# basilevh/tcow

Hardware: AMD Instinct MI355X
Metric: train clips/sec (T=30, 240x320) (higher is better)
Workload: dtype bf16; 1 GPU; TCOW Seeker train step: T=30 240x320 patch16, 12-layer divided space-time ViT (D=768), num_queries=3, causal_attention=1, 1 clip/GPU; clips_per_gpu=1, num_queries=3, parallelism=dp1, optimizer=AdamW lr 1e-4, clip 0.3

## Files before the change

### tcow_amd/csrc/gemm_bf16.hip

```cpp
#include <stdlib.h>

#include "common.h"
#include "gemm_nt_common.h"

namespace {

constexpr int BM = 128, BN = 128;
constexpr int BK = 64;
constexpr int TILE_BYTES = BM * 128;
constexpr int STAGE_BYTES = 2 * TILE_BYTES;
constexpr int NT_LDS_BYTES = 2 * STAGE_BYTES;

__device__ __forceinline__ void nt_epilogue(const NtParams& p, char* smem, f32x16 (&acc)[2][2], float4 b4, int tid, int wm, int wn, int l31, int hi, int m0, int n0) {
    const int c4 = (tid & 31) * 4, gn = n0 + c4;
    const bool col_ok = gn < p.N;
    float* ct = reinterpret_cast<float*>(smem);
#pragma unroll
    for (int i = 0; i < 2; ++i)
#pragma unroll
        for (int j = 0; j < 2; ++j)
#pragma unroll
            for (int r = 0; r < 16; ++r) {
                const int row = wm * 64 + i * 32 + crow32(r, hi);
                const int col = wn * 64 + j * 32 + l31;
// ... 584 lines not shown
    const int mbeg = z * p.mps;
    const int mend = (mbeg + p.mps < p.M) ? mbeg + p.mps : p.M;

    const int lrow = lane >> 5, cl = lane & 31;
    const bf16_t* zero = reinterpret_cast<const bf16_t*>(&g_zero16);
    int ycol[2], xcol[2];
#pragma unroll
    for (int e = 0; e < 2; ++e) {
        const int r3 = (e << 1) | lrow;
        const int sc = cl ^ (r3 << 2);
        ycol[e] = n0 + sc * 8; xcol[e] = k0 + sc * 8;
    }
    f32x16 acc[4][2];
#pragma unroll
    for (int i = 0; i < 4; ++i)
#pragma unroll
        for (int j = 0; j < 2; ++j)
#pragma unroll
            for (int r = 0; r < 16; ++r) acc[i][j][r] = 0.f;

    auto issue = [&](int mt, int stage) {
        char* sy = smem + stage * T2_STAGE;
        char* sx = sy + T2_TILE;
#pragma unroll
        for (int j = 0; j < 4; ++j) {
            const int q = wave * 4 + j;
            const int gm = mt + q * 2 + lrow;
            const bool ok = gm < mend;
            const bf16_t* ys = (ok && ycol[j & 1] < p.N) ? p.dY + (size_t)gm * p.ldy + ycol[j & 1] : zero;
            const bf16_t* xs = (ok && xcol[j & 1] < p.K) ? p.X + (size_t)gm * p.ldx + xcol[j & 1] : zero;
            glds16(ys, sy + q * 1024);
            glds16(xs, sx + q * 1024);
        }
    };
    const bool interior = n0 + T2 <= p.N && k0 + T2 <= p.K;
    typedef int i32x4_ __attribute__((ext_vector_type(4)));
    auto make_srd = [](const void* base, long bytes) {
        const uint64_t b = (uint64_t)(uintptr_t)base;
        i32x4_ r; r[0] = (int)(uint32_t)b; r[1] = (int)(uint32_t)((b >> 32) & 0xffffu); r[2] = (int)(uint32_t)bytes; r[3] = 0x00020000;
        return r;
    };
    const i32x4_ srd_y = make_srd(p.dY, ((long)(p.M - 1) * p.ldy + p.N) * 2), srd_x = make_srd(p.X, ((long)(p.M - 1) * p.ldx + p.K) * 2);
    const uint32_t yv0 = (uint32_t)(lrow * p.ldy + ycol[0]) * 2u, yv1 = (uint32_t)(lrow * p.ldy + ycol[1]) * 2u;
    const uint32_t xv0 = (uint32_t)(lrow * p.ldx + xcol[0]) * 2u, xv1 = (uint32_t)(lrow * p.ldx + xcol[1]) * 2u;
    const bool small32 = (long)p.M * p.ldy < (1L << 29) && (long)p.M * p.ldx < (1L << 29);
    const uint32_t lds_base = (uint32_t)(uintptr_t)(LDS_PTR(char))smem;
#define TN_BLD(voff, srd, soff, ldsdst) \
    asm volatile("s_mov_b32 m0, %3\n\ts_nop 0\n\tbuffer_load_dwordx4 %0, %1, %2 offen lds" :: "v"(voff), "s"(srd), "s"(soff), "s"(ldsdst) : "memory")
    auto issue_fast = [&](int mt, int stage) {
        const uint32_t dy = lds_base + stage * T2_STAGE + wave * 4096, dx = dy + T2_TILE;
        const uint32_t sy = (uint32_t)((long)(mt + wave * 8) * p.ldy * 2), sx = (uint32_t)((long)(mt + wave * 8) * p.ldx * 2);
        const uint32_t ry = (uint32_t)(2 * p.ldy * 2), rx = (uint32_t)(2 * p.ldx * 2);
        TN_BLD(yv0, srd_y, sy, dy); TN_BLD(xv0, srd_x, sx, dx);
        TN_BLD(yv1, srd_y, sy + ry, dy + 1024); TN_BLD(xv1, srd_x, sx + rx, dx + 1024);
        TN_BLD(yv0, srd_y, sy + 2 * ry, dy + 2048); TN_BLD(xv0, srd_x, sx + 2 * rx, dx + 2048);
        TN_BLD(yv1, srd_y, sy + 3 * ry, dy + 3072); TN_BLD(xv1, srd_x, sx + 3 * rx, dx + 3072);
    };
    const int q16 = lane & 15, g16 = (lane >> 4) & 1, hi = lane >> 5;
    const int rr = 8 * hi + (q16 >> 2);
    int y_off[4], x_off[2];
#pragma unroll
    for (int i = 0; i < 4; ++i) {
        const int cy = wm * 128 + i * 32 + 16 * g16 + 4 * (q16 & 3);
        y_off[i] = rr * T2_ROWB + ((((cy >> 3) ^ ((q16 >> 2) << 2))) << 4) + (cy & 7) * 2;
    }
#pragma unroll
    for (int j = 0; j < 2; ++j) {
        const int cx = wn * 64 + j * 32 + 16 * g16 + 4 * (q16 & 3);
        x_off[j] = rr * T2_ROWB + ((((cx >> 3) ^ ((q16 >> 2) << 2))) << 4) + (cx & 7) * 2;
    }

    const int cs_col = tid & 255;
    const int cs_lo = pk * p.rows_per_pk, cs_hi = (cs_lo + p.rows_per_pk < T2_MC) ? cs_lo + p.rows_per_pk : T2_MC;
    const int cs_chunk = tid & 31, cs_rg = tid >> 5;
    float csum[8] = {0.f, 0.f, 0.f, 0.f, 0.f, 0.f, 0.f, 0.f};

    const int nmt = (mend - mbeg + T2_MC - 1) / T2_MC;
    auto issue_stage = [&](int st_, int buf_) {
        const int mt = mbeg + st_ * T2_MC;
        if (interior && small32 && (mt + T2_MC <= mend || mend == p.M)) issue_fast(mt, buf_); else issue(mt, buf_);
    };
    if constexpr (SCHED >= 2) {
        if (nmt > 0) {
            issue_fast(mbeg, 0);
            if (nmt > 1) { issue_fast(mbeg + T2_MC, 1); asm volatile("s_waitcnt vmcnt(8)" ::: "memory"); }
            else asm volatile("s_waitcnt vmcnt(0)" ::: "memory");
            __syncthreads();
        }
    } else if (nmt > 0) {
        issue(mbeg, 0);
        if (SCHED == 1 && nmt > 1) { issue_stage(1, 1); asm volatile("s_waitcnt vmcnt(8)" ::: "memory"); }
        else asm volatile("s_waitcnt vmcnt(0)" ::: "memory");
        __syncthreads();
    }
    typedef uint32_t u32x2 __attribute__((ext_vector_type(2)));
    typedef uint32_t u32x4 __attribute__((ext_vector_type(4)));
    const uint32_t lds0 = (uint32_t)(uintptr_t)(LDS_PTR(char))smem;
    uint32_t ya[4], xa[2];
#pragma unroll
    for (int i = 0; i < 4; ++i) ya[i] = lds0 + (uint32_t)y_off[i];
#pragma unroll
    for (int j = 0; j < 2; ++j) xa[j] = lds0 + (uint32_t)x_off[j];
    u32x2 fyl[2][4], fyh[2][4], fxl[2][2], fxh[2][2];
    u32x4 kfrag = (u32x4){1u, 2u, 3u, 4u};
    if (AB & 128) asm volatile("" : "+v"(kfrag));
    u32x4 kfy[2][4], kfx[2][2];
    if (AB & 512) {
#pragma unroll
        for (int b = 0; b < 2; ++b) {
#pragma unroll
            for (int i = 0; i < 4; ++i) {
                kfy[b][i] = (u32x4){1u, 2u, 3u, 4u};
                if (AB & 1024) {
#pragma unroll
                    for (int c = 0; c < 4; ++c) { uint32_t h = (uint32_t)(tid * 97 + b * 31 + i * 7 + c) * 2654435761u; kfy[b][i][c] = (h & 0x807f807fu) | 0x3f003f00u | ((h >> 3) & 0x00800080u); }
                }
                asm volatile("" : "+v"(kfy[b][i]));
            }
#pragma unroll
            for (int j = 0; j < 2; ++j) {
                kfx[b][j] = (u32x4){1u, 2u, 3u, 4u};
                if (AB & 1024) {
#pragma unroll
                    for (int c = 0; c < 4; ++c) { uint32_t h = (uint32_t)(tid * 89 + b * 29 + j * 5 + c + 1000) * 2654435761u; kfx[b][j][c] = (h & 0x807f807fu) | 0x3f003f00u | ((h >> 3) & 0x00800080u); }
                }
                asm volatile("" : "+v"(kfx[b][j]));
            }
        }
    }
#define TCOW_TRR(dst, addr, off) asm volatile("ds_read_b64_tr_b16 %0, %1 offset:%2" : "=v"(dst) : "v"(addr), "i"(off))
#define TCOW_TN_READ(buf, ks, so)                                                                                          \
    do {                                                                                                                   \
        if (AB & 16) break;                                                                                                \
        _Pragma("unroll") for (int j = 0; j < 2; ++j) {                                                                    \
            TCOW_TRR(fxl[buf][j], xa[j] + (so), T2_TILE + (ks) * 16 * T2_ROWB);                                            \
            TCOW_TRR(fxh[buf][j], xa[j] + (so), T2_TILE + (ks) * 16 * T2_ROWB + 4 * T2_ROWB);                              \
        }                                                                                                                  \
        _Pragma("unroll") for (int i = 0; i < 4; ++i) {                                                                    \
            TCOW_TRR(fyl[buf][i], ya[i] + (so), (ks) * 16 * T2_ROWB);                                                      \
            TCOW_TRR(fyh[buf][i], ya[i] + (so), (ks) * 16 * T2_ROWB + 4 * T2_ROWB);                                        \
        }                                                                                                                  \
    } while (0)
#define TCOW_TN_FRAG(lo, hi) ((AB & 128) ? __builtin_bit_cast(bf16x8, kfrag) : __builtin_bit_cast(bf16x8, (u32x4){(lo).x, (lo).y, (hi).x, (hi).y}))
#define TCOW_TN_MFMA8(buf)                                                                                                 \
    if (!(AB & 32)) _Pragma("unroll") for (int i = 0; i < 4; ++i)                                                          \
        _Pragma("unroll") for (int j = 0; j < 2; ++j)                                                                      \
            acc[i][j] = TCOW_MFMA_32x32x16_H16(TCOW_TN_FRAG(fyl[buf][i], fyh[buf][i]), TCOW_TN_FRAG(fxl[buf][j], fxh[buf][j]), acc[i][j], 0, 0, 0)

    if (nmt > 0) TCOW_TN_READ(0, 0, 0u);
    if (AB & 16) {
#pragma unroll
        for (int b = 0; b < 2; ++b) {
#pragma unroll
            for (int j = 0; j < 2; ++j) { fxl[b][j] = (u32x2){1u, 2u}; fxh[b][j] = (u32x2){3u, 4u}; }
#pragma unroll
            for (int i = 0; i < 4; ++i) { fyl[b][i] = (u32x2){5u, 6u}; fyh[b][i] = (u32x2){7u, 8u}; }
        }
    }
    if constexpr (SCHED == 2) {
#define TN_BLDA(...) do { if (!(AB & 2)) TN_BLD(__VA_ARGS__); } while (0)
#define TN_RDA(...) do { if (!(AB & 16)) TCOW_TRR(__VA_ARGS__); } while (0)
#define TN_NOP do { } while (0)
#define TN_MF(cur, i, j) if (!(AB & 32)) acc[i][j] = TCOW_MFMA_32x32x16_H16((AB & 512) ? __builtin_bit_cast(bf16x8, kfy[cur][i]) : TCOW_TN_FRAG(fyl[cur][i], fyh[cur][i]), (AB & 512) ? __builtin_bit_cast(bf16x8, kfx[cur][j]) : TCOW_TN_FRAG(fxl[cur][j], fxh[cur][j]), acc[i][j], 0, 0, 0); \
                    __builtin_amdgcn_sched_barrier(0)
#define TN_BLK(cur, nxt, OFFK, son, W0, B0, B1, B2, B3, B4, B5, B6, B7)                                                                  \
    do {                                                                                                                                 \
        if (!(AB & 256)) asm volatile("s_waitcnt lgkmcnt(" #W0 ")" ::: "memory"); __builtin_amdgcn_sched_barrier(0);                     \
        TN_MF(cur, 0, 0); TN_RDA(fxl[nxt][0], xa[0] + (son), T2_TILE + (OFFK)); TN_RDA(fxh[nxt][0], xa[0] + (son), T2_TILE + (OFFK) + 4 * T2_ROWB); B0; \
        TN_MF(cur, 0, 1); TN_RDA(fxl[nxt][1], xa[1] + (son), T2_TILE + (OFFK)); TN_RDA(fxh[nxt][1], xa[1] + (son), T2_TILE + (OFFK) + 4 * T2_ROWB); B1; \
        TN_MF(cur, 1, 0); TN_RDA(fyl[nxt][0], ya[0] + (son), (OFFK)); TN_RDA(fyh[nxt][0], ya[0] + (son), (OFFK) + 4 * T2_ROWB); B2;              \
        TN_MF(cur, 1, 1); TN_RDA(fyl[nxt][1], ya[1] + (son), (OFFK)); TN_RDA(fyh[nxt][1], ya[1] + (son), (OFFK) + 4 * T2_ROWB); B3;              \
        if (!(AB & 256)) asm volatile("s_waitcnt lgkmcnt(10)" ::: "memory"); __builtin_amdgcn_sched_barrier(0);     \
        TN_MF(cur, 2, 0); TN_RDA(fyl[nxt][2], ya[2] + (son), (OFFK)); TN_RDA(fyh[nxt][2], ya[2] + (son), (OFFK) + 4 * T2_ROWB); B4;              \
        TN_MF(cur, 2, 1); TN_RDA(fyl[nxt][3], ya[3] + (son), (OFFK)); TN_RDA(fyh[nxt][3], ya[3] + (son), (OFFK) + 4 * T2_ROWB); B5;              \
        if (!(AB & 256)) asm volatile("s_waitcnt lgkmcnt(12)" ::: "memory"); __builtin_amdgcn_sched_barrier(0);      \
        TN_MF(cur, 3, 0); B6;                                                                                                            \
        TN_MF(cur, 3, 1); B7;                                                                                                            \
    } while (0)
        for (int it = 0; it < nmt; ++it) {
            const int stage = it & 1;
            const uint32_t so = (uint32_t)stage * T2_STAGE;
            const char* sy = smem + stage * T2_STAGE;
            TN_BLK(0, 1, 1 * 16 * T2_ROWB, so, 4, TN_NOP, TN_NOP, TN_NOP, TN_NOP, TN_NOP, TN_NOP, TN_NOP, TN_NOP);
            TN_BLK(1, 0, 2 * 16 * T2_ROWB, so, 4, TN_NOP, TN_NOP, TN_NOP, TN_NOP, TN_NOP, TN_NOP, TN_NOP, TN_NOP);
            TN_BLK(0, 1, 3 * 16 * T2_ROWB, so, 4, TN_NOP, TN_NOP, TN_NOP, TN_NOP, TN_NOP, TN_NOP, TN_NOP, TN_NOP);
            if (p.bias_part && !(AB & 64)) {
#pragma unroll
                for (int u = 0; u < 4; ++u) {
                    const int r = cs_lo + cs_rg + 16 * u;
                    if (r < cs_hi) {
                        const uint4 v = *reinterpret_cast<const uint4*>(sy + r * T2_ROWB + ((cs_chunk ^ ((r & 3) << 2)) << 4));
                        csum[0] += bflo(v.x); csum[1] += bfhi(v.x); csum[2] += bflo(v.y); csum[3] += bfhi(v.y);
                        csum[4] += bflo(v.z); csum[5] += bfhi(v.z); csum[6] += bflo(v.w); csum[7] += bfhi(v.w);
                    }
                }
            }
            asm volatile("s_waitcnt vmcnt(0) lgkmcnt(0)" ::: "memory");
            if (!(AB & 4)) __syncthreads();
            {
                const int mt2 = mbeg + (it + 2) * T2_MC;
                const bool more = it + 2 < nmt;
                const uint32_t dy = lds_base + so + wave * 4096, dx = dy + T2_TILE;
                const uint32_t by = (uint32_t)((long)(mt2 + wave * 8) * p.ldy * 2), bx = (uint32_t)((long)(mt2 + wave * 8) * p.ldx * 2);
                const uint32_t yw0 = more ? yv0 : 0x80000000u, yw1 = more ? yv1 : 0x80000000u;
                const uint32_t xw0 = more ? xv0 : 0x80000000u, xw1 = more ? xv1 : 0x80000000u;
                const uint32_t ry = (uint32_t)(2 * p.ldy * 2), rx = (uint32_t)(2 * p.ldx * 2);
                const uint32_t sn = so ^ (uint32_t)T2_STAGE;
                TN_BLK(1, 0, 0, sn, 0, TN_BLDA(yw0, srd_y, by, dy), TN_BLDA(xw0, srd_x, bx, dx), TN_BLDA(yw1, srd_y, by + ry, dy + 1024),
                       TN_BLDA(xw1, srd_x, bx + rx, dx + 1024), TN_BLDA(yw0, srd_y, by + 2 * ry, dy + 2048), TN_BLDA(xw0, srd_x, bx + 2 * rx, dx + 2048),
                       TN_BLDA(yw1, srd_y, by + 3 * ry, dy + 3072), TN_BLDA(xw1, srd_x, bx + 3 * rx, dx + 3072));
            }
        }
#undef TN_BLK
#undef TN_MF
#undef TN_NOP
#undef TN_BLDA
#undef TN_RDA
    } else
    if constexpr (SCHED == 1) {
        for (int it = 0; it < nmt; ++it) {
            const int stage = it & 1;
            const uint32_t so = (uint32_t)stage * T2_STAGE;
            const char* sy = smem + stage * T2_STAGE;
            TCOW_TN_READ(1, 1, so);
            asm volatile("s_waitcnt lgkmcnt(12)" ::: "memory");
            __builtin_amdgcn_sched_barrier(0);
            TCOW_TN_MFMA8(0);
            TCOW_TN_READ(0, 2, so);
            asm volatile("s_waitcnt lgkmcnt(12)" ::: "memory");
            __builtin_amdgcn_sched_barrier(0);
            TCOW_TN_MFMA8(1);
            TCOW_TN_READ(1, 3, so);
            asm volatile("s_waitcnt lgkmcnt(12)" ::: "memory");
            __builtin_amdgcn_sched_barrier(0);
            TCOW_TN_MFMA8(0);
            if (p.bias_part && !(AB & 64)) {
#pragma unroll
                for (int u = 0; u < 4; ++u) {
                    const int r = cs_lo + cs_rg + 16 * u;
                    if (r < cs_hi) {
                        const uint4 v = *reinterpret_cast<const uint4*>(sy + r * T2_ROWB + ((cs_chunk ^ ((r & 3) << 2)) << 4));
                        csum[0] += bflo(v.x); csum[1] += bfhi(v.x); csum[2] += bflo(v.y); csum[3] += bfhi(v.y);
                        csum[4] += bflo(v.z); csum[5] += bfhi(v.z); csum[6] += bflo(v.w); csum[7] += bfhi(v.w);
                    }
                }
            }
            asm volatile("s_waitcnt vmcnt(0) lgkmcnt(0)" ::: "memory");
            if (!(AB & 4)) __syncthreads();
            if (it + 2 < nmt && !(AB & 2)) issue_stage(it + 2, stage);
            if (it + 1 < nmt) TCOW_TN_READ(0, 0, so ^ (uint32_t)T2_STAGE);
            __builtin_amdgcn_sched_barrier(0);
            TCOW_TN_MFMA8(1);
        }
    }
    asm volatile("s_waitcnt lgkmcnt(0)"
                 : "+v"(fxl[0][0]), "+v"(fxl[0][1]), "+v"(fxh[0][0]), "+v"(fxh[0][1]), "+v"(fyl[0][0]), "+v"(fyl[0][1]), "+v"(fyl[0][2]), "+v"(fyl[0][3]),
                   "+v"(fyh[0][0]), "+v"(fyh[0][1]), "+v"(fyh[0][2]), "+v"(fyh[0][3])
                 :: "memory");
    __builtin_amdgcn_sched_barrier(0);
#undef TCOW_TRR
#undef TCOW_TN_READ
#undef TCOW_TN_FRAG
#undef TCOW_TN_MFMA8
    if (p.bias_part) {
        float* red = reinterpret_cast<float*>(smem);
        __syncthreads();
#pragma unroll
        for (int e = 0; e < 8; ++e) red[cs_rg * 256 + cs_chunk * 8 + e] = csum[e];
        __syncthreads();
        if (n0 + cs_col < p.N) {
            float t = 0.f;
            if (tid < 256) {
#pragma unroll
                for (int g = 0; g < 16; ++g) t += red[g * 256 + cs_col];
            }
            p.bias_part[(((size_t)z * p.tiles_k + pk) * 2 + (tid >> 8)) * p.N + n0 + cs_col] = t;
        }
        __syncthreads();
    }

    if (AB & 8) {
#pragma unroll
        for (int i = 0; i < 4; ++i)
#pragma unroll
            for (int j = 0; j < 2; ++j) asm volatile("" :: "v"(acc[i][j]));
        return;
    }
    float* out = p.slab + (size_t)z * p.N * p.K;
    const int l31 = lane & 31;
#pragma unroll
    for (int i = 0; i < 4; ++i)
#pragma unroll
        for (int j = 0; j < 2; ++j) {
            const int gk = k0 + wn * 64 + j * 32 + l31;
            if (gk >= p.K) continue;
#pragma unroll
            for (int r = 0; r < 16; ++r) {
                const int gn = n0 + wm * 128 + i * 32 + crow32(r, hi);
                if (gn < p.N) out[(size_t)gn * p.K + gk] = acc[i][j][r];
            }
        }
}

template <int SCHED>
__global__ __launch_bounds__(512, 2) void gemm_tn_bf16_256_kernel(TnParams p) {
    extern __shared__ __attribute__((aligned(16))) char smem[];
    tn256_body<0, SCHED>(p, xcd_remap(blockIdx.x, gridDim.x), smem);
}

constexpr int TN_GROUP_MAX = 40;
struct TnGroup { int n; int first[TN_GROUP_MAX + 1]; TnParams p[TN_GROUP_MAX]; };
template <int SCHED>
__global__ __launch_bounds__(512, 2) void gemm_tn_bf16_256_group_kernel(TnGroup g) {
    extern __shared__ __attribute__((aligned(16))) char smem[];
    const int pid = xcd_remap(blockIdx.x, gridDim.x);
    int k = 0;
    while (k + 1 < g.n && pid >= g.first[k + 1]) ++k;
    const TnParams p = g.p[k];
    tn256_body<0, SCHED>(p, pid - g.first[k], smem);
}

}

int tcow_tn_splits_256(int M, int N, int K) {
    const int tiles = cdiv(N, T2) * cdiv(K, T2);
    int s = 256 / tiles;
    const int max_s = M / 256;
    if (s > max_s) s = max_s;
    if (s > 64) s = 64;
    if (s < 1) s = 1;
    return s;
}
bool tcow_tn_use_256(int M, int N, int K) {
    const int tiles = cdiv(N, T2) * cdiv(K, T2);
    return M >= 4096 && N >= 256 && K >= 256 && tiles >= 9 && tiles <= 256;
}

static int tn_sched() { return 2; }
static bool tn_whole(int M, int N, int K, long ldy, long ldx) { return N % T2 == 0 && K % T2 == 0 && (long)M * ldy < (1L << 29) && (long)M * ldx < (1L << 29); }

int tcow_gemm_tn_bf16(hipStream_t stream, int M, int N, int K, const bf16_t* dY, long ldy, const bf16_t* X, long ldx, float* slab, int splits,
                      int* nz_out, float* bias_part, int* bias_parts_out) {
    TCOW_CHECK_ARG(N % 8 == 0 && K % 8 == 0 && ldy % 8 == 0 && ldx % 8 == 0, "tcow_gemm_tn(bf16): N, K, ldy, ldx must be multiples of 8");
    TnParams p;
    p.M = M; p.N = N; p.K = K; p.dY = dY; p.ldy = ldy; p.X = X; p.ldx = ldx; p.slab = slab;
    p.tiles_n = cdiv(N, TN_T); p.tiles_k = cdiv(K, TN_T);
    constexpr int mc = 32;
    int mps = cdiv(M, splits); mps = ((mps + 63) / 64) * 64;
    p.mps = mps;
    const int nz = cdiv(M, mps);
    p.nz = nz;
    *nz_out = nz;
    p.bias_part = bias_part;
    p.rows_per_pk = cdiv(mc, p.tiles_k);
    if (bias_parts_out) *bias_parts_out = nz * p.tiles_k * 2;
    if (tcow_tn_use_256(M, N, K)) {
        p.tiles_n = cdiv(N, T2); p.tiles_k = cdiv(K, T2);
        p.rows_per_pk = cdiv(T2_MC, p.tiles_k);
        if (bias_parts_out) *bias_parts_out = nz * p.tiles_k * 2;
        const int sched = (tn_sched() >= 2 && !tn_whole(M, N, K, ldy, ldx)) ? 1 : tn_sched();
#define TN_LAUNCH(S)                                                                                                       \
    do {                                                                                                                   \
        tcow_ensure_lds(reinterpret_cast<const void*>(gemm_tn_bf16_256_kernel<S>), T2_LDS);                                \
        hipLaunchKernelGGL(gemm_tn_bf16_256_kernel<S>, dim3(nz * p.tiles_n * p.tiles_k), dim3(512), T2_LDS, stream, p);    \
    } while (0)
        if (sched == 2) TN_LAUNCH(2); else TN_LAUNCH(1);
#undef TN_LAUNCH
        TCOW_CHECK_LAUNCH();
        return TCOW_OK;
    }
    const dim3 grid(8 * cdiv(nz, 8) * p.tiles_n * p.tiles_k);
    hipLaunchKernelGGL(gemm_tn_bf16_kernel<32>, grid, dim3(256), 32768, stream, p);
    TCOW_CHECK_LAUNCH();
    return TCOW_OK;
}

int tcow_tn_group_max(void) { return TN_GROUP_MAX; }
bool tcow_tn_group_ok(int n, const tcow_tn_problem* pr) {
    if (n < 2 || n > TN_GROUP_MAX) return false;
    for (int i = 0; i < n; ++i) {
        if (pr[i].M != pr[0].M || !tcow_tn_use_256(pr[i].M, pr[i].N, pr[i].K)) return false;
        if (pr[i].N % 8 || pr[i].K % 8 || pr[i].ldy % 8 || pr[i].ldx % 8) return false;
    }
    return true;
}
int tcow_tn_group_slices(int n, const tcow_tn_problem* pr) {
    int tiles = 0;
    for (int i = 0; i < n; ++i) tiles += cdiv(pr[i].N, T2) * cdiv(pr[i].K, T2);
    int max_s = pr[0].M / 256; if (max_s > 64) max_s = 64; if (max_s < 1) max_s = 1;
    int best = 1; double best_cost = 1e30;
    for (int s = 1; s <= max_s; ++s) {
        const int wg = s * tiles, rounds = cdiv(wg, 256);
        const double cost = (rounds * 256.0) / (double)wg + 0.044 * s;
        if (cost < best_cost - 1e-9) { best_cost = cost; best = s; }
    }
    return best;
}
int tcow_gemm_tn_bf16_group(hipStream_t stream, int n, const tcow_tn_problem* pr, int nz_req, float* const* slabs, float* const* bias_parts, int* nz_out,
                            int* bias_nparts) {
    TnGroup g;
    g.n = n;
    int first = 0, nz = 0;
    for (int i = 0; i < n; ++i) {
        TnParams& p = g.p[i];
        p.M = pr[i].M; p.N = pr[i].N; p.K = pr[i].K; p.dY = (const bf16_t*)pr[i].dY; p.ldy = pr[i].ldy; p.X = (const bf16_t*)pr[i].X; p.ldx = pr[i].ldx;
        p.slab = slabs[i];
        p.tiles_n = cdiv(p.N, T2); p.tiles_k = cdiv(p.K, T2);
        int mps = cdiv(p.M, nz_req); mps = ((mps + 63) / 64) * 64;
        p.mps = mps; p.nz = cdiv(p.M, mps); nz = p.nz;
        p.bias_part = bias_parts[i];
        p.rows_per_pk = cdiv(T2_MC, p.tiles_k);
        bias_nparts[i] = p.nz * p.tiles_k * 2;
        g.first[i] = first;
        first += p.nz * p.tiles_n * p.tiles_k;
    }
    g.first[n] = first;
    for (int i = n + 1; i <= TN_GROUP_MAX; ++i) g.first[i] = first;
    *nz_out = nz;
    int sched = tn_sched();
    for (int i = 0; i < n && sched >= 2; ++i) if (!tn_whole(pr[i].M, pr[i].N, pr[i].K, pr[i].ldy, pr[i].ldx)) sched = 1;
#define TN_LAUNCH(S)                                                                                                       \
    do {                                                                                                                   \
        tcow_ensure_lds(reinterpret_cast<const void*>(gemm_tn_bf16_256_group_kernel<S>), T2_LDS);                          \
        hipLaunchKernelGGL(gemm_tn_bf16_256_group_kernel<S>, dim3(first), dim3(512), T2_LDS, stream, g);                   \
    } while (0)
    if (sched == 2) TN_LAUNCH(2); else TN_LAUNCH(1);
#undef TN_LAUNCH
    TCOW_CHECK_LAUNCH();
    return TCOW_OK;
}
```

Measured before the change: 36.72 clips/s.

## Add phased ping-pong schedule for 256-tile TN weight-gradient GEMM

Adds a new tn256_phased body for the weight-gradient (TN) GEMM. It splits each K-stage into four phases that interleave transposed LDS reads (ds_read_b64_tr_b16), buffer loads for the next stage and 16x16x32 MFMA bursts. The two wave groups are staggered by an extra barrier, and the MFMA bursts run at raised priority. The default schedule switches from 2 to 3, so all whole-tile TN launches use it. This is meant to overlap memory and matrix work better than the old body, at the cost of heavier barrier choreography and a fragile vmcnt-based ordering.

Result: no change. 36.81 clips/s (median of 6 runs) (+0.2%).

```diff
diff --git a/tcow_amd/csrc/gemm_bf16.hip b/tcow_amd/csrc/gemm_bf16.hip
--- a/tcow_amd/csrc/gemm_bf16.hip
+++ b/tcow_amd/csrc/gemm_bf16.hip
@@ -910,10 +910,222 @@
         }
 }
 
+template <int AB>
+__device__ __forceinline__ void tn256_phased(const TnParams& p, const int pid, char* smem) {
+    const int tid = threadIdx.x, lane = tid & 63;
+    const int wave = __builtin_amdgcn_readfirstlane(tid >> 6);
+    const int wm = wave >> 2, wn = wave & 3;
+    const int ntile = p.tiles_n * p.tiles_k;
+    const int z = pid / ntile, tile = pid - z * ntile;
+    const int pn = tile / p.tiles_k, pk = tile - pn * p.tiles_k;
+    const int n0 = pn * T2, k0 = pk * T2;
+    const int mbeg = z * p.mps;
+    const int mend = (mbeg + p.mps < p.M) ? mbeg + p.mps : p.M;
+    const int nmt = (mend - mbeg + T2_MC - 1) / T2_MC;
+
+    typedef int i32x4_ __attribute__((ext_vector_type(4)));
+    typedef uint32_t u32x2 __attribute__((ext_vector_type(2)));
+    typedef uint32_t u32x4 __attribute__((ext_vector_type(4)));
+    auto make_srd = [](const void* base, long bytes) {
+        const uint64_t b = (uint64_t)(uintptr_t)base;
+        i32x4_ r; r[0] = (int)(uint32_t)b; r[1] = (int)(uint32_t)((b >> 32) & 0xffffu); r[2] = (int)(uint32_t)bytes; r[3] = 0x00020000;
+        return r;
+    };
+    const i32x4_ srd_y = make_srd(p.dY, ((long)(p.M - 1) * p.ldy + p.N) * 2), srd_x = make_srd(p.X, ((long)(p.M - 1) * p.ldx + p.K) * 2);
+    const int lrow = lane >> 5, cl = lane & 31;
+    uint32_t yv[2], xv[2];
+#pragma unroll
+    for (int e = 0; e < 2; ++e) {
+        const int sc = cl ^ ((2 * e + lrow + 4 * ((wave >> 1) & 1)) << 1);
+        yv[e] = (uint32_t)(lrow * p.ldy + n0 + sc * 8) * 2u;
+        xv[e] = (uint32_t)(lrow * p.ldx + k0 + sc * 8) * 2u;
+    }
+    const uint32_t lds0 = (uint32_t)(uintptr_t)(LDS_PTR(char))smem;
+    const uint32_t ryw = (uint32_t)(4 * wave * p.ldy * 2), rxw = (uint32_t)(4 * wave * p.ldx * 2);
+    const uint32_t ry2 = (uint32_t)(2 * p.ldy * 2), rx2 = (uint32_t)(2 * p.ldx * 2), ry32 = (uint32_t)(32 * p.ldy * 2), rx32 = (uint32_t)(32 * p.ldx * 2);
+    auto load_q = [&](int st, int buf, bool more, int h, int e) {
+        if (AB & 2) return;
+        const int mt = mbeg + st * T2_MC;
+        const uint32_t by = (uint32_t)((long)mt * p.ldy * 2) + ryw + h * ry32 + e * ry2;
+        const uint32_t bx = (uint32_t)((long)mt * p.ldx * 2) + rxw + h * rx32 + e * rx2;
+        const uint32_t dy = lds0 + buf * T2_STAGE + (32 * h + 4 * wave + 2 * e) * T2_ROWB, dx = dy + T2_TILE;
+        TN_BLD(more ? yv[e] : 0x80000000u, srd_y, by, dy);
+        TN_BLD(more ? xv[e] : 0x80000000u, srd_x, bx, dx);
+    };
+    const int q16 = lane & 15, g4 = lane >> 4;
+    const int trow = 8 * g4 + (q16 >> 2);
+    const int swz = (trow & 3) | ((trow >> 1) & 4);
+    uint32_t xa[4], ya[8];
+#pragma unroll
+    for (int j = 0; j < 4; ++j) xa[j] = lds0 + T2_TILE + trow * T2_ROWB + (((wn * 4 + j) ^ swz) << 5) + (q16 & 3) * 8;
+#pragma unroll
+    for (int i = 0; i < 8; ++i) ya[i] = lds0 + trow * T2_ROWB + (((wm * 8 + i) ^ swz) << 5) + (q16 & 3) * 8;
+
+    const int cs_col = tid & 255;
+    const int cs_lo = pk * p.rows_per_pk, cs_hi = (cs_lo + p.rows_per_pk < T2_MC) ? cs_lo + p.rows_per_pk : T2_MC;
+    const int cs_chunk = tid & 31, cs_rg = tid >> 5;
+    float csum[8] = {0.f, 0.f, 0.f, 0.f, 0.f, 0.f, 0.f, 0.f};
+
+    f32x4 acc[8][4];
+#pragma unroll
+    for (int i = 0; i < 8; ++i)
+#pragma unroll
+        for (int j = 0; j < 4; ++j) acc[i][j] = (f32x4){0.f, 0.f, 0.f, 0.f};
+    u32x2 fxl[2][4], fxh[2][4], fyl[2][4], fyh[2][4];
+    if (AB & 16) {
+#pragma unroll
+        for (int b = 0; b < 2; ++b)
+#pragma unroll
+            for (int i = 0; i < 4; ++i) {
+                u32x4 vx = (u32x4){1u, 2u, 3u, 4u}, vy = (u32x4){5u, 6u, 7u, 8u};
+                if (AB & 1024) {
+#pragma unroll
+                    for (int c = 0; c < 4; ++c) {
+                        const uint32_t hx = (uint32_t)(tid * 89 + b * 29 + i * 5 + c + 1000) * 2654435761u, hy = (uint32_t)(tid * 97 + b * 31 + i * 7 + c) * 2654435761u;
+                        vx[c] = (hx & 0x807f807fu) | 0x3f003f00u | ((hx >> 3) & 0x00800080u);
+                        vy[c] = (hy & 0x807f807fu) | 0x3f003f00u | ((hy >> 3) & 0x00800080u);
+                    }
+                }
+                asm volatile("" : "+v"(vx), "+v"(vy));
+                fxl[b][i] = (u32x2){vx[0], vx[1]}; fxh[b][i] = (u32x2){vx[2], vx[3]};
+                fyl[b][i] = (u32x2){vy[0], vy[1]}; fyh[b][i] = (u32x2){vy[2], vy[3]};
+            }
+    }
+#define TN3_TRR(dst, addr, off) asm volatile("ds_read_b64_tr_b16 %0, %1 offset:%2" : "=v"(dst) : "v"(addr), "i"(off))
+#define TN3_READ_X(b, so, h)                                                                                               \
+    do {                                                                                                                   \
+        if (AB & 16) break;                                                                                                \
+        _Pragma("unroll") for (int j = 0; j < 4; ++j) {                                                                    \
+            TN3_TRR(fxl[b][j], xa[j] + (so), (h) * 32 * T2_ROWB);                                                          \
+            TN3_TRR(fxh[b][j], xa[j] + (so), (h) * 32 * T2_ROWB + 4 * T2_ROWB);                                            \
+        }                                                                                                                  \
+    } while (0)
+#define TN3_READ_Y(b, so, h)                                                                                               \
+    do {                                                                                                                   \
+        if (AB & 16) break;                                                                                                \
+        _Pragma("unroll") for (int i = 0; i < 4; ++i) {                                                                    \
+            TN3_TRR(fyl[b][i], ya[4 * (b) + i] + (so), (h) * 32 * T2_ROWB);                                                \
+            TN3_TRR(fyh[b][i], ya[4 * (b) + i] + (so), (h) * 32 * T2_ROWB + 4 * T2_ROWB);                                  \
+        }                                                                                                                  \
+    } while (0)
+#define TN3_FRAG(lo, hi) __builtin_bit_cast(bf16x8, (u32x4){(lo).x, (lo).y, (hi).x, (hi).y})
+#define TN3_TAIL(h, nh)                                                                                                    \
+    do {                                                                                                                   \
+        if (!(AB & 4)) __builtin_amdgcn_s_barrier();                                                                       \
+        asm volatile("s_waitcnt lgkmcnt(0)" ::: "memory");                                                                 \
+        __builtin_amdgcn_sched_barrier(0);                                                                                 \
+        if (!(AB & 32)) {                                                                                                  \
+            __builtin_amdgcn_s_setprio(1);                                                                                 \
+            _Pragma("unroll") for (int i = 0; i < 4; ++i)                                                                  \
+                _Pragma("unroll") for (int j = 0; j < 4; ++j)                                                              \
+                    acc[4 * (nh) + i][j] = TCOW_MFMA_16x16x32_H16(TN3_FRAG(fxl[h][j], fxh[h][j]), TN3_FRAG(fyl[nh][i], fyh[nh][i]), \
+                                                                  acc[4 * (nh) + i][j], 0, 0, 0);                                  \
+            __builtin_amdgcn_s_setprio(0);                                                                                 \
+        }                                                                                                                  \
+        __builtin_amdgcn_sched_barrier(0);                                                                                 \
+        if (!(AB & 4)) __builtin_amdgcn_s_barrier();                                                                       \
+    } while (0)
+
+    if (nmt > 0) {
+        const uint32_t by = (uint32_t)((long)mbeg * p.ldy * 2) + ryw, bx = (uint32_t)((long)mbeg * p.ldx * 2) + rxw;
+#pragma unroll
+        for (int q = 0; q < 4; ++q) {
+            const int h = q >> 1, e = q & 1;
+            const uint32_t dy = lds0 + (32 * h + 4 * wave + 2 * e) * T2_ROWB;
+            TN_BLD(yv[e], srd_y, by + h * ry32 + e * ry2, dy);
+            TN_BLD(xv[e], srd_x, bx + h * rx32 + e * rx2, dy + T2_TILE);
+        }
+        asm volatile("s_waitcnt vmcnt(0)" ::: "memory");
+    }
+    if (!(AB & 4)) {
+        __builtin_amdgcn_s_barrier();
+        if (wm == 1) __builtin_amdgcn_s_barrier();
+    }
+    for (int it = 0; it < nmt; ++it) {
+        const int buf = it & 1;
+        const uint32_t so = (uint32_t)buf * T2_STAGE;
+        const bool more = it + 1 < nmt;
+        TN3_READ_X(0, so, 0); TN3_READ_Y(0, so, 0);
+        load_q(it + 1, buf ^ 1, more, 0, 0);
+        TN3_TAIL(0, 0);
+        TN3_READ_Y(1, so, 0);
+        load_q(it + 1, buf ^ 1, more, 0, 1);
+        asm volatile("s_waitcnt vmcnt(4)" ::: "memory");
+        TN3_TAIL(0, 1);
+        TN3_READ_X(1, so, 1); TN3_READ_Y(0, so, 1);
+        load_q(it + 1, buf ^ 1, more, 1, 0);
+        TN3_TAIL(1, 0);
+        if (p.bias_part && !(AB & 64)) {
+            const char* sy = smem + buf * T2_STAGE;
+#pragma unroll
+            for (int u = 0; u < 4; ++u) {
+                const int r = cs_lo + cs_rg + 16 * u;
+                if (r < cs_hi) {
+                    const int sw = (r & 3) | ((r >> 1) & 4);
+                    const uint4 v = *reinterpret_cast<const uint4*>(sy + r * T2_ROWB + ((cs_chunk ^ (sw << 1)) << 4));
+                    csum[0] += bflo(v.x); csum[1] += bfhi(v.x); csum[2] += bflo(v.y); csum[3] += bfhi(v.y);
+                    csum[4] += bflo(v.z); csum[5] += bfhi(v.z); csum[6] += bflo(v.w); csum[7] += bfhi(v.w);
+                }
+            }
+        }
+        __builtin_amdgcn_sched_barrier(0);
+        TN3_READ_Y(1, so, 1);
+        load_q(it + 1, buf ^ 1, more, 1, 1);
+        asm volatile("s_waitcnt vmcnt(4)" ::: "memory");
+        TN3_TAIL(1, 1);
+    }
+    if (wm == 0 && !(AB & 4)) __builtin_amdgcn_s_barrier();
+    asm volatile("s_waitcnt vmcnt(0) lgkmcnt(0)"
+                 : "+v"(fxl[0][0]), "+v"(fxl[0][1]), "+v"(fxl[0][2]), "+v"(fxl[0][3]), "+v"(fxh[0][0]), "+v"(fxh[0][1]), "+v"(fxh[0][2]), "+v"(fxh[0][3]),
+                   "+v"(fxl[1][0]), "+v"(fxl[1][1]), "+v"(fxl[1][2]), "+v"(fxl[1][3]), "+v"(fxh[1][0]), "+v"(fxh[1][1]), "+v"(fxh[1][2]), "+v"(fxh[1][3])
+                 :: "memory");
+    asm volatile(""
+                 : "+v"(fyl[0][0]), "+v"(fyl[0][1]), "+v"(fyl[0][2]), "+v"(fyl[0][3]), "+v"(fyh[0][0]), "+v"(fyh[0][1]), "+v"(fyh[0][2]), "+v"(fyh[0][3]),
+                   "+v"(fyl[1][0]), "+v"(fyl[1][1]), "+v"(fyl[1][2]), "+v"(fyl[1][3]), "+v"(fyh[1][0]), "+v"(fyh[1][1]), "+v"(fyh[1][2]), "+v"(fyh[1][3])
+                 :: "memory");
+    __builtin_amdgcn_sched_barrier(0);
+#undef TN3_TRR
+#undef TN3_READ_X
+#undef TN3_READ_Y
+#undef TN3_FRAG
+#undef TN3_TAIL
+    if (p.bias_part) {
+        float* red = reinterpret_cast<float*>(smem);
+        __syncthreads();
+#pragma unroll
+        for (int e = 0; e < 8; ++e) red[cs_rg * 256 + cs_chunk * 8 + e] = csum[e];
+        __syncthreads();
+        if (n0 + cs_col < p.N) {
+            float t = 0.f;
+            if (tid < 256) {
+#pragma unroll
+                for (int g = 0; g < 16; ++g) t += red[g * 256 + cs_col];
+            }
+            p.bias_part[(((size_t)z * p.tiles_k + pk) * 2 + (tid >> 8)) * p.N + n0 + cs_col] = t;
+        }
+        __syncthreads();
+    }
+    if (AB & 8) {
+#pragma unroll
+        for (int i = 0; i < 8; ++i)
+#pragma unroll
+            for (int j = 0; j < 4; ++j) asm volatile("" :: "v"(acc[i][j]));
+        return;
+    }
+    float* out = p.slab + (size_t)z * p.N * p.K;
+#pragma unroll
+    for (int i = 0; i < 8; ++i) {
+        const size_t gn = (size_t)(n0 + wm * 128 + i * 16 + q16);
+#pragma unroll
+        for (int j = 0; j < 4; ++j) *reinterpret_cast<f32x4*>(out + gn * p.K + k0 + wn * 64 + j * 16 + 4 * g4) = acc[i][j];
+    }
+}
+
 template <int SCHED>
 __global__ __launch_bounds__(512, 2) void gemm_tn_bf16_256_kernel(TnParams p) {
     extern __shared__ __attribute__((aligned(16))) char smem[];
-    tn256_body<0, SCHED>(p, xcd_remap(blockIdx.x, gridDim.x), smem);
+    if constexpr (SCHED == 3) tn256_phased<0>(p, xcd_remap(blockIdx.x, gridDim.x), smem);
+    else tn256_body<0, SCHED>(p, xcd_remap(blockIdx.x, gridDim.x), smem);
 }
 
 constexpr int TN_GROUP_MAX = 40;
@@ -925,7 +1137,8 @@
     int k = 0;
     while (k + 1 < g.n && pid >= g.first[k + 1]) ++k;
     const TnParams p = g.p[k];
-    tn256_body<0, SCHED>(p, pid - g.first[k], smem);
+    if constexpr (SCHED == 3) tn256_phased<0>(p, pid - g.first[k], smem);
+    else tn256_body<0, SCHED>(p, pid - g.first[k], smem);
 }
 
 }
@@ -944,7 +1157,7 @@
     return M >= 4096 && N >= 256 && K >= 256 && tiles >= 9 && tiles <= 256;
 }
 
-static int tn_sched() { return 2; }
+static int tn_sched() { return 3; }
 static bool tn_whole(int M, int N, int K, long ldy, long ldx) { return N % T2 == 0 && K % T2 == 0 && (long)M * ldy < (1L << 29) && (long)M * ldx < (1L << 29); }
 
 int tcow_gemm_tn_bf16(hipStream_t stream, int M, int N, int K, const bf16_t* dY, long ldy, const bf16_t* X, long ldx, float* slab, int splits,
@@ -972,7 +1185,7 @@
         tcow_ensure_lds(reinterpret_cast<const void*>(gemm_tn_bf16_256_kernel<S>), T2_LDS);                                \
         hipLaunchKernelGGL(gemm_tn_bf16_256_kernel<S>, dim3(nz * p.tiles_n * p.tiles_k), dim3(512), T2_LDS, stream, p);    \
     } while (0)
-        if (sched == 2) TN_LAUNCH(2); else TN_LAUNCH(1);
+        if (sched == 3) TN_LAUNCH(3); else TN_LAUNCH(1);
 #undef TN_LAUNCH
         TCOW_CHECK_LAUNCH();
         return TCOW_OK;
@@ -1032,7 +1245,7 @@
         tcow_ensure_lds(reinterpret_cast<const void*>(gemm_tn_bf16_256_group_kernel<S>), T2_LDS);                          \
         hipLaunchKernelGGL(gemm_tn_bf16_256_group_kernel<S>, dim3(first), dim3(512), T2_LDS, stream, g);                   \
     } while (0)
-    if (sched == 2) TN_LAUNCH(2); else TN_LAUNCH(1);
+    if (sched == 3) TN_LAUNCH(3); else TN_LAUNCH(1);
 #undef TN_LAUNCH
     TCOW_CHECK_LAUNCH();
     return TCOW_OK;
```
